# crowsonkb/style_transfer

Hardware: AMD Instinct MI355X
Metric: tile-iterations/sec, VGG-19 2048px/1024-tile (fwd+bwd, Gram/content losses, regularizers, Adam step) (higher is better)
Workload: dtype f32 (fp16x2-split MFMA, fp32 accumulate)

## Files before the change

### style_transfer_amd/build.py

```python

import concurrent.futures
import os
import subprocess
import sys

CSRC = os.path.join(os.path.dirname(os.path.abspath(__file__)), 'csrc')
REPO = os.path.dirname(os.path.dirname(os.path.abspath(__file__)))
INCLUDE = os.path.join(REPO, 'include')
LIB = os.path.join(CSRC, 'libstx.so')
HIPCC = os.environ.get('HIPCC', '/opt/rocm/bin/hipcc')
ARCH = 'gfx950'

SOURCES = {
    'conv_mfma.hip': [],
    'conv_wino2.hip': [],
    'conv_first.hip': [],
    'conv_h2.hip': [],
    'gram.hip': [],
    'symm.hip': [],
    'pool.hip': [],
    'reduce.hip': [],
    'content_mask.hip': [],
    'image_ops.hip': ['-ffp-contract=off'],
    'swt.hip': ['-ffp-contract=off'],
    'style_mask.hip': ['-ffp-contract=off'],
    'lap.hip': ['-ffp-contract=off'],
    'stat.hip': ['-ffp-contract=off'],
    'conv_dispatch.cpp': [],
    'engine.cpp': [],
    'tile_path.cpp': [],
    'image_api.cpp': [],
    'op_hooks.cpp': [],
}
EXTRA = os.environ.get('STX_HIPCC_EXTRA', '').split()
COMMON = EXTRA + ['--offload-arch=' + ARCH, '-O3', '-std=c++17', '-fPIC', '-I' + INCLUDE, '-I' + CSRC,
          '-Wall', '-Wno-unused-function']


def _stale(target, deps):
    if not os.path.exists(target):
        return True
    t = os.path.getmtime(target)
    return any(os.path.getmtime(d) > t for d in deps)


def _compile(src, extra, force):
    obj = os.path.join(CSRC, os.path.splitext(src)[0] + '.o')
    path = os.path.join(CSRC, src)
    deps = [path, os.path.join(CSRC, 'common.h'), os.path.join(CSRC, 'bf16x3.h'),
            os.path.join(CSRC, 'f16x2.h'), os.path.join(CSRC, 'engine.h'), os.path.join(INCLUDE, 'stx.h')]
    if force or _stale(obj, deps):
        cmd = [HIPCC] + COMMON + extra + ['-c', path, '-o', obj]
        proc = subprocess.run(cmd, stdout=subprocess.PIPE, stderr=subprocess.STDOUT, text=True)
        if proc.returncode != 0:
            raise RuntimeError('hipcc failed on %s:\n%s' % (src, proc.stdout))
        if proc.stdout.strip():
            sys.stderr.write(proc.stdout)
    return obj


def build(force=False, verbose=False):
    with concurrent.futures.ThreadPoolExecutor(max_workers=len(SOURCES)) as ex:
        futs = [ex.submit(_compile, src, extra, force) for src, extra in SOURCES.items()]
        objs = [f.result() for f in futs]
    if force or _stale(LIB, objs):
        cmd = [HIPCC, '--offload-arch=' + ARCH, '-shared', '-fPIC', '-o', LIB] + objs
        proc = subprocess.run(cmd, stdout=subprocess.PIPE, stderr=subprocess.STDOUT, text=True)
        if proc.returncode != 0:
            raise RuntimeError('link failed:\n' + proc.stdout)
    if verbose:
        print('built', LIB)
    return LIB


if __name__ == '__main__':
    build(force='--force' in sys.argv, verbose=True)
```

### style_transfer_amd/csrc/common.h

```cpp
#pragma once

#include <hip/hip_runtime.h>

#include <vector>

#include <cstdarg>
#include <cstdio>
#include <functional>
#include <string>

#include "stx.h"

namespace stx {

constexpr float kEps = 1.1920928955078125e-07f;

void set_error(const char *fmt, ...);

const char *sw_env(const char *name);
void sw_reread();

#define STX_HIP(call)                                                                       \
    do {                                                                                    \
        hipError_t err__ = (call);                                                          \
// ... 205 lines not shown
int wino2_splitk_factor(const ConvConfig &cfg, const ConvProblem &p);
struct Wino2Tail { int items, slices; };
Wino2Tail wino2_tail_split(const ConvConfig &cfg, const ConvProblem &p);
int wino2_max_slices(const ConvConfig &cfg, const ConvProblem &p);

constexpr int kAmaxSlots = 64;
ConvConfig h2_config(int mb, int pb = 1);
ConvConfig h2_pick_config(const ConvProblem &p);
bool h2_usable(const ConvProblem &p);
size_t h2_packed_floats(int K, int M);
int h2_pack_weights(hipStream_t s, const float *w_caffe, int Mo, int Ko, int transpose_flip, float *packed);
int h2_launch(hipStream_t s, const ConvConfig &cfg, const ConvProblem &p, int ksplit);
int h2_splitk_factor(const ConvConfig &cfg, const ConvProblem &p);
bool h2_fuses_pool(const ConvProblem &p);
bool h2_takes_pooled_input(const ConvConfig &cfg, const ConvProblem &p);
int absmax_launch(hipStream_t s, const float *x, size_t n, unsigned *slots);

size_t conv_small_packed_floats(int K);
int conv_small_pack(hipStream_t s, const float *w_caffe, int Mo, int Ko, int transpose_flip,
                    float *packed);
int conv_small_launch(hipStream_t s, const float *x, const float *packed, float *y,
                      const float *mask, int K, int M, int H, int W);

bool conv_h2_enabled();
struct ConvTuner { int device; hipStream_t stream; hipEvent_t ev0, ev1; std::function<int(const ConvConfig &, const float **)> bank; };
int conv_choose(const ConvProblem &p, bool winograd, const ConvTuner *tuner, ConvConfig *out);
struct ConvBank { int key; size_t floats; std::function<int(hipStream_t, const float *w_caffe, float *packed)> pack; };
ConvBank conv_bank(const ConvConfig &cfg, int dir, int Mo, int Ko, int ksize);
ConvBank conv_small_bank(int Mo, int Ko);
int conv_dispatch(hipStream_t s, const ConvConfig &cfg, const ConvProblem &p, double *flop_algorithmic,
                  double *flop_issued);
int conv_splitk_factor(const ConvConfig &cfg, const ConvProblem &p);
size_t conv_splitk_floats(const ConvConfig &cfg, const ConvProblem &p);
bool conv_takes_clock(const ConvConfig &cfg);
bool conv_fuses_pool(const ConvConfig &cfg, const ConvProblem &p);
bool conv_writes_pool_codes(const ConvConfig &cfg);
bool conv_reads_x_amax(const ConvConfig &cfg);
bool conv_leaves_y_amax(const ConvConfig &cfg);
bool conv_takes_inject(const ConvConfig &cfg);
bool conv_takes_pooled_input(const ConvConfig &cfg, const ConvProblem &p);
bool conv_uses_relu_codes(const ConvConfig &cfg, const ConvProblem &p, int ksplit);
bool conv_writes_out_codes(const ConvConfig &cfg, const ConvProblem &p, int ksplit);

int pool_forward_launch(hipStream_t s, const float *x, int C, int H, int W, int mode, float *y,
                        unsigned char *codes = nullptr);
int pool_backward_codes_launch(hipStream_t s, const float *dy, const unsigned char *codes, int C,
                               int H, int W, int mode, bool relu_mask, float *dx);
int pool_backward_launch(hipStream_t s, const float *dy, const float *x, int C, int H, int W,
                         int mode, bool relu_mask, float *dx);

struct GramPlan {
    int C, HW, splits, tiles;
    int parts;
    size_t partial_floats;
};
GramPlan gram_plan(int C, int HW);
bool gram_h2_usable(const float *feat, int C, int HW);
int gram_partials_launch(hipStream_t s, const float *feat, const GramPlan &plan, float *partials,
                         const unsigned *f_amax = nullptr);
int gram_finish_blocks(const GramPlan &plan);
int gram_finish_launch(hipStream_t s, const float *partials, const GramPlan &plan, float *gram_out,
                       const float *target, float *dsym, float *sumsq, unsigned short *pieces = nullptr,
                       const unsigned *f_amax = nullptr, float *block_out = nullptr);

size_t symm_pieces_elems(int C);
int symm_num_workgroups(int C, int HW);
bool symm_bf3_usable(const float *feat, const float *out, int C, int HW);
bool symm_h2_usable(const float *feat, const float *out, int C, int HW);
int symm_h2_launch(hipStream_t s, const float *feat, const float *dsym, const unsigned *d_amax, int n_damax,
                   const unsigned *f_amax, float *out, float *partials, int C, int HW);
int symm_bf3_launch(hipStream_t s, const float *feat, const float *dsym, unsigned short *pieces,
                    bool pieces_ready, float *out, float *partials, int C, int HW);

#ifdef __HIPCC__
__device__ __forceinline__ int content_origin_y(const ContentWindow &w) { return w.oy - w.sy; }
__device__ __forceinline__ int content_origin_x(const ContentWindow &w) { return w.ox - w.sx; }
__device__ __forceinline__ size_t content_index(const ContentWindow &w, int c, int y, int x) {
    int yy = (content_origin_y(w) + y) % w.ch;
    int xx = (content_origin_x(w) + x) % w.cw;
    if (yy < 0) yy += w.ch;
    if (xx < 0) xx += w.cw;
    return ((size_t)c * w.ch + yy) * w.cw + xx;
}
#endif

struct SumJob {
    const float *src;
    int n;
    float *dst;
};
int sum_jobs_launch(hipStream_t s, const SumJob *jobs, int n_jobs);
int content_sums_launch(hipStream_t s, const float *feat, const float *content,
                        const ContentWindow &win, float *sums , std::vector<SumJob> *defer = nullptr);
int inject_style_launch(hipStream_t s, float *diff, const float *sgrad, size_t n,
                        const float *abs_sum, float coef, bool accumulate, unsigned *y_amax = nullptr);
int inject_content_launch(hipStream_t s, float *diff, const float *feat, const float *content,
                          const ContentWindow &win, const float *sums, float coef, bool accumulate,
                          unsigned *y_amax = nullptr);
int relu_inplace_launch(hipStream_t s, float *x, size_t n);
int sum_partials_launch(hipStream_t s, const float *partials, int n, float *out);
int sum_partials2_launch(hipStream_t s, const float *a, int na, float *out_a, const float *b, int nb,
                         float *out_b);

constexpr int kMaskParts = 1024;
constexpr int kMaskSgradParts = 2048;
int mask_map_launch(hipStream_t s, const float *mask, int H, int W, int scale, float *out);
int mask_apply_launch(hipStream_t s, const float *feat, const float *map, const ContentWindow &win, float *fm,
                      float *m2_partials, int *n_parts);
int mask_target_launch(hipStream_t s, const float *gs, int C, const float *m2_partials, int n_parts, int HW,
                       float *out, float *a_out);
int mask_sgrad_launch(hipStream_t s, float *sgrad, const float *map, const ContentWindow &win, const float *a,
                      float *partials, int *n_parts);

constexpr int kContentMaskParts = 1024;
int content_mask_mean_launch(hipStream_t s, const float *map, const ContentWindow &win, float *a_out);
int content_mask_term_launch(hipStream_t s, const float *feat, const float *content, const float *map,
                             const ContentWindow &win, const float *a, float *sgrad, float *partials,
                             int *n_parts);

constexpr int kStatSlice = 16384;
constexpr float kStatEps = 1e-5f;
// ... 82 lines not shown
```

### style_transfer_amd/csrc/gram.hip

```cpp

#include <algorithm>
#include <cstdlib>
#include <cstring>

#include "bf16x3.h"
#include "common.h"
#include "f16x2.h"

namespace stx {

typedef float f32x16 __attribute__((ext_vector_type(16)));

constexpr int kGT = 64;
constexpr int kGP = 64;
constexpr int kGLd = kGP + 1;

GramPlan gram_plan(int C, int HW) {
    GramPlan p;
    p.C = C;
    p.HW = HW;
    const int T = ceil_div(C, kGT);
    p.tiles = T * (T + 1) / 2;
    int target = 512, min_stages = 8;
    if (const char *env = sw_env("STX_GRAM_WGS")) target = std::max(1, atoi(env));
    if (const char *env = sw_env("STX_GRAM_MIN_STAGES")) min_stages = std::max(1, atoi(env));
    int splits = std::max(1, target / p.tiles);
    splits = std::min(splits, ceil_div(HW, min_stages * kGP));
    splits = std::max(splits, 1);
    p.splits = splits;
    p.parts = 1;
    p.partial_floats = (size_t)p.splits * p.parts * p.tiles * kGT * kGT;
    return p;
}

__device__ __forceinline__ void tile_coords(int tile, int &ti, int &tj) {
    int r = (int)((sqrtf(8.f * tile + 1.f) - 1.f) * 0.5f);
    while ((r + 1) * (r + 2) / 2 <= tile) ++r;
    while (r * (r + 1) / 2 > tile) --r;
    ti = r;
    tj = tile - r * (r + 1) / 2;
}

template <bool VEC4>
__global__ __launch_bounds__(256, 2) void gram_partial_kernel(const float *__restrict__ F, int C,
                                                              int HW, int tiles, int slice,
                                                              int parts,
                                                              float *__restrict__ partials) {
    __shared__ float At[kGT * kGLd];
    __shared__ float Bt[kGT * kGLd];
    const int tid = threadIdx.x, lane = tid & 63;
    const int wave = __builtin_amdgcn_readfirstlane(tid >> 6);
    const int l31 = lane & 31, half = lane >> 5;
    const int tile = blockIdx.x % tiles, split = blockIdx.x / tiles;
    int ti, tj;
    tile_coords(tile, ti, tj);
    const bool diag = ti == tj;
    const int p_begin = split * slice;
    const int p_end = min(HW, p_begin + slice);
    const int bi = wave >> 1, bj = wave & 1;

    f32x16 acc;
#pragma unroll
    for (int r = 0; r < 16; ++r) acc[r] = 0.f;

    float ra[16], rb[16];
    auto load = [&](int p0) {
        if (VEC4) {
#pragma unroll
            for (int n = 0; n < 4; ++n) {
                const int e = tid + 256 * n;
                const int ch = e >> 4, px = p0 + (e & 15) * 4;
                const int ca = ti * kGT + ch, cb = tj * kGT + ch;
                const bool okp = px < p_end;
                const bool oka = okp && ca < C, okb = okp && cb < C && !diag;
                const float4 va = *reinterpret_cast<const float4 *>(F + (oka ? (size_t)ca * HW + px : 0));
                const float4 vb = *reinterpret_cast<const float4 *>(F + (okb ? (size_t)cb * HW + px : 0));
                ra[4 * n + 0] = oka ? va.x : 0.f;
                ra[4 * n + 1] = oka ? va.y : 0.f;
                ra[4 * n + 2] = oka ? va.z : 0.f;
                ra[4 * n + 3] = oka ? va.w : 0.f;
                rb[4 * n + 0] = okb ? vb.x : 0.f;
                rb[4 * n + 1] = okb ? vb.y : 0.f;
                rb[4 * n + 2] = okb ? vb.z : 0.f;
                rb[4 * n + 3] = okb ? vb.w : 0.f;
            }
        } else {
#pragma unroll
            for (int n = 0; n < 16; ++n) {
                const int e = tid + 256 * n;
                const int ch = e >> 6, px = p0 + (e & 63);
                const int ca = ti * kGT + ch, cb = tj * kGT + ch;
                const bool okp = px < p_end;
                const bool oka = okp && ca < C, okb = okp && cb < C && !diag;
// ... 420 lines not shown
        if (p_begin + kGP < p_end) load(p_begin + kGP);
        __syncthreads();
        int buf = 0;
        for (int p0 = p_begin; p0 < p_end; p0 += kGP, buf ^= 1) {
            const float *base = lds + buf * kStageFloats;
            f16x8h ah[2], al[2], bh[2], bl[2];
            fragment(base + a_off, ah[0], al[0]);
            fragment(base + a_off + 32 * kGLdW, ah[1], al[1]);
            if (!diag) {
                fragment(base + b_off, bh[0], bl[0]);
                fragment(base + b_off + 32 * kGLdW, bh[1], bl[1]);
            }
            if (p0 + kGP < p_end) store(p0 + kGP, buf ^ 1);
            if (p0 + 2 * kGP < p_end) load(p0 + 2 * kGP);
#pragma unroll
            for (int i = 0; i < 2; ++i)
#pragma unroll
                for (int j = 0; j < 2; ++j) {
                    if (diag && j > i) continue;
                    acc[i][j] = mfma_split3(ah[i], al[i], diag ? ah[j] : bh[j], diag ? al[j] : bl[j], acc[i][j]);
                }
            __syncthreads();
        }
    }
    float *red = lds + wave * (kGT * kGT);
#pragma unroll
    for (int i = 0; i < 2; ++i)
#pragma unroll
        for (int j = 0; j < 2; ++j)
#pragma unroll
            for (int r = 0; r < 16; ++r) {
                const int row = i * 32 + (r & 3) + 8 * (r >> 2) + 4 * half;
                red[row * kGT + j * 32 + l31] = acc[i][j][r];
            }
    __syncthreads();
    static_assert(4 * kGT * kGT <= 2 * kStageFloats, "the four partial tiles must fit the stage buffers");
    float *out = partials + ((size_t)split * tiles + tile) * (kGT * kGT);
#pragma unroll
    for (int n = 0; n < 4; ++n) {
        const int e = tid + 256 * n;
        const float4 w0 = reinterpret_cast<const float4 *>(lds)[e];
        const float4 w1 = reinterpret_cast<const float4 *>(lds + kGT * kGT)[e];
        const float4 w2 = reinterpret_cast<const float4 *>(lds + 2 * kGT * kGT)[e];
        const float4 w3 = reinterpret_cast<const float4 *>(lds + 3 * kGT * kGT)[e];
        float4 v;
        v.x = ((w0.x + w1.x) + w2.x) + w3.x;
        v.y = ((w0.y + w1.y) + w2.y) + w3.y;
        v.z = ((w0.z + w1.z) + w2.z) + w3.z;
        v.w = ((w0.w + w1.w) + w2.w) + w3.w;
        reinterpret_cast<float4 *>(out)[e] = v;
    }
}

static bool gram_use_bf3() {
    const char *env = sw_env("STX_GRAM");
    return !(env && !strcmp(env, "fp32"));
}

bool gram_h2_usable(const float *feat, int C, int HW) {
    const char *env = sw_env("STX_GRAM");
    if (env && (!strcmp(env, "fp32") || !strcmp(env, "bf3"))) return false;
    return (reinterpret_cast<uintptr_t>(feat) & 3) == 0 && 4.0 * C * (double)HW < 2147483648.0;
}

int gram_partials_launch(hipStream_t s, const float *feat, const GramPlan &plan, float *partials,
                         const unsigned *f_amax) {
    int slice = ceil_div(plan.HW, plan.splits);
    slice = ceil_div(slice, kGP) * kGP;
    const bool aligned = (reinterpret_cast<uintptr_t>(feat) & 15) == 0;
    const double bytes = 4.0 * plan.C * (double)plan.HW;
    if (f_amax) {
        gram_partial_h2_kernel<<<plan.tiles * plan.splits, 256, 0, s>>>(
            feat, plan.C, plan.HW, plan.tiles, slice, (unsigned)bytes, f_amax, partials);
        STX_CHECK_LAUNCH();
        return STX_OK;
    }
    if ((reinterpret_cast<uintptr_t>(feat) & 3) == 0 && bytes < 2147483648.0 && gram_use_bf3()) {
        gram_partial_bf3_kernel<<<plan.tiles * plan.splits, 256, 0, s>>>(
            feat, plan.C, plan.HW, plan.tiles, slice, (unsigned)bytes, partials);
        STX_CHECK_LAUNCH();
        return STX_OK;
    }
    if ((reinterpret_cast<uintptr_t>(feat) & 3) == 0 && bytes < 2147483648.0 && !sw_env("STX_GRAM_NARROW")) {
        gram_partial_wide_kernel<<<plan.tiles * plan.splits, 256, 0, s>>>(
            feat, plan.C, plan.HW, plan.tiles, slice, (unsigned)bytes, partials);
        STX_CHECK_LAUNCH();
        return STX_OK;
    }
    if (plan.parts > 1)
        STX_HIP(hipMemsetAsync(partials, 0, plan.partial_floats * sizeof(float), s));
    if (plan.HW % 4 == 0 && aligned)
        gram_partial_kernel<true><<<plan.tiles * plan.splits, 256, 0, s>>>(
            feat, plan.C, plan.HW, plan.tiles, slice, plan.parts, partials);
    else
        gram_partial_kernel<false><<<plan.tiles * plan.splits, 256, 0, s>>>(
            feat, plan.C, plan.HW, plan.tiles, slice, plan.parts, partials);
    STX_CHECK_LAUNCH();
    return STX_OK;
}

__global__ __launch_bounds__(256) void gram_finish_kernel(const float *__restrict__ partials, int C,
                                                          int tiles, int splits, float scale,
                                                          float *__restrict__ gram,
                                                          const float *__restrict__ target,
                                                          float *__restrict__ dsym,
                                                          float *__restrict__ block_sumsq,
                                                          unsigned short *__restrict__ pieces,
                                                          const unsigned *__restrict__ f_amax,
                                                          unsigned *__restrict__ block_amax) {
    __shared__ float lane_sum[4][64];
    __shared__ float red[64];
    __shared__ float redm[64];
    float unscale = 1.f;
    if (f_amax) unscale = pow2f(-h2_scale_exp(amax_of_slots(f_amax, kAmaxSlots)));
    const int el = threadIdx.x & 63, sl = threadIdx.x >> 6;
    const int idx = blockIdx.x * 64 + el;
    const bool valid = idx < C * C;
    int i = 0, j = 0;
    float sum = 0.f;
    if (valid) {
        i = idx / C;
        j = idx % C;
    }
// ... 156 lines not shown
```

### style_transfer_amd/csrc/symm.hip

```cpp

#include <algorithm>
#include <cstdlib>
#include <cstring>

#include "bf16x3.h"
#include "common.h"
#include "f16x2.h"

#ifndef STX_SYMM_SKIP
#define STX_SYMM_SKIP 0
#endif

namespace stx {

namespace {

constexpr int kSM = 64;
constexpr int kSN = 256;
#ifndef STX_SYMM_KSK
#define STX_SYMM_KSK 32
#endif
constexpr int kSK = STX_SYMM_KSK;
constexpr int kSPC = kSK / 16;
constexpr int kSegs = kSK / 8;
// ... 132 lines not shown
                acc[i][j] = mfma_split6(pa[i], pb[j], acc[i][j]);
            }
    };

    int step = 0;
    auto advance = [&](int slot_) {
        const int chunk = step / kSPC, s_in = step % kSPC, buf = chunk & 1;
        if (step + kRing - 1 < n_steps && !(STX_SYMM_SKIP & 4)) f_load(step + kRing - 1, (slot_ + kRing - 1) % kRing);
        do_step(step, slot_, buf, s_in);
        if (s_in == kSPC - 1) {
            if (chunk + 1 < n_chunks) d_store(buf ^ 1);
            if (chunk + 2 < n_chunks) d_load(chunk + 2);
            __syncthreads();
        }
        ++step;
    };
    while (step < n_steps) {
#pragma unroll
        for (int r = 0; r < kRing; ++r)
            if (step < n_steps) advance(r);
    }

    float asum = 0.f;
#pragma unroll
    for (int i = 0; i < 2; ++i)
#pragma unroll
        for (int r = 0; r < 16; ++r) {
            const int row = m0 + i * 32 + (r & 3) + 8 * (r >> 2) + 4 * g;
            const int row0 = min(__builtin_amdgcn_readfirstlane(m0 + i * 32 + (r & 3) + 8 * (r >> 2)), C);
            const unsigned so = BIG ? 0u : (unsigned)row0 * HW4;
            const int rows_left = C - row0 < 5 ? C - row0 : 5;
            const __amdgpu_buffer_rsrc_t rrow =
                BIG ? __builtin_amdgcn_make_buffer_rsrc(S + (size_t)row0 * (size_t)HW, 0,
                                                        (rows_left > 0 ? rows_left : 0) * HW * 4, 0x00020000)
                    : rs;
#pragma unroll
            for (int j = 0; j < 2; ++j) {
                const int px = px0 + j * 32 + l31;
                const bool ok = row < C && px < HW;
                const float v = acc[i][j][r];
                asum += ok ? fabsf(v) : 0.f;
                const unsigned vo = ok ? (unsigned)((4 * g) * HW + px) * 4u : kOob;
                if (!(STX_SYMM_SKIP & 8))
                    __builtin_amdgcn_raw_buffer_store_b32(__builtin_bit_cast(unsigned, v), rrow, vo, so, 0);
            }
        }
#pragma unroll
    for (int off = 32; off > 0; off >>= 1) asum += __shfl_down(asum, off, 64);
    if (lane == 0) wave_sum[wave] = asum;
    __syncthreads();
    if (tid == 0) partials[blockIdx.x] = ((wave_sum[0] + wave_sum[1]) + wave_sum[2]) + wave_sum[3];
}

constexpr int kHChunkBytes = 2 * kPieceBytes;
constexpr int kHDLoads = kSM * kSK / 4 / 256;

template <bool BIG>
__global__ __launch_bounds__(256, 2) void symm_h2_kernel(const float *__restrict__ F,
                                                         const float *__restrict__ D,
                                                         const unsigned *__restrict__ d_amax, int n_damax,
                                                         const unsigned *__restrict__ f_amax,
                                                         float *__restrict__ S,
                                                         float *__restrict__ partials, int C, int Cp,
                                                         int HW, unsigned f_bytes, int m_tiles) {
    __shared__ __attribute__((aligned(16))) unsigned char lds[2 * kHChunkBytes];
    __shared__ float wave_sum[4];
    __shared__ unsigned wave_max[4];
    const int tid = threadIdx.x, lane = tid & 63;
    const int wave = __builtin_amdgcn_readfirstlane(tid >> 6);
    const int l31 = lane & 31, g = lane >> 5;
    const int nb = gridDim.x, xcd = blockIdx.x & 7, slot = blockIdx.x >> 3;
    const int q8 = nb >> 3, r8 = nb & 7;
    const int L = (xcd < r8 ? xcd * (q8 + 1) : r8 * (q8 + 1) + (xcd - r8) * q8) + slot;
    const int mt = __builtin_amdgcn_readfirstlane(L % m_tiles), pt = __builtin_amdgcn_readfirstlane(L / m_tiles);
    const int m0 = mt * kSM;
    const int px0 = pt * kSN + wave * 64;

    constexpr unsigned kOob = 0x80000000u;
    const __amdgpu_buffer_rsrc_t rf =
        __builtin_amdgcn_make_buffer_rsrc(const_cast<float *>(F), 0, BIG ? 0 : f_bytes, 0x00020000);
    const __amdgpu_buffer_rsrc_t rs = __builtin_amdgcn_make_buffer_rsrc(S, 0, BIG ? 0 : f_bytes, 0x00020000);
    const __amdgpu_buffer_rsrc_t rd =
        __builtin_amdgcn_make_buffer_rsrc(const_cast<float *>(D), 0, (unsigned)(C * C) * 4u, 0x00020000);
    unsigned voff[2];
#pragma unroll
    for (int j = 0; j < 2; ++j) {
        const int px = px0 + j * 32 + l31;
        voff[j] = px < HW ? (unsigned)((g * 8) * HW + px) * 4u : kOob;
    }
    const unsigned HW4 = (unsigned)HW * 4u;
    const int n_steps = Cp / 16, n_chunks = Cp / kSK;

    unsigned dvoff[kHDLoads], ddst[kHDLoads];
    int dcol[kHDLoads];
#pragma unroll
    for (int n = 0; n < kHDLoads; ++n) {
        const int e = tid + 256 * n;
        const int row = e / (kSK / 4), seg = e - row * (kSK / 4);
        dcol[n] = seg * 4;
        dvoff[n] = m0 + row < C ? (unsigned)((m0 + row) * C + seg * 4) * 4u : kOob;
        ddst[n] = (unsigned)(row * kRowBytes + seg * 8);
    }
    u32x4y dreg[kHDLoads];
    auto d_load = [&](int chunk) {
        const unsigned so = (unsigned)__builtin_amdgcn_readfirstlane(chunk * kSK * 4);
#pragma unroll
        for (int n = 0; n < kHDLoads; ++n)
            dreg[n] = __builtin_amdgcn_raw_buffer_load_b128(rd, dcol[n] + chunk * kSK < C ? dvoff[n] : kOob, so, 0);
    };

    float raw[kRing][2][8];
    auto f_load = [&](int step, int slot_) {
        const int k0 = __builtin_amdgcn_readfirstlane(step * 16);
        const int left = C - k0 < 16 ? C - k0 : 16;
        const __amdgpu_buffer_rsrc_t rk =
            BIG ? __builtin_amdgcn_make_buffer_rsrc(const_cast<float *>(F) + (size_t)k0 * (size_t)HW, 0,
                                                    (left > 0 ? left : 0) * HW * 4, 0x00020000)
                : rf;
#pragma unroll
        for (int j = 0; j < 2; ++j)
#pragma unroll
            for (int e = 0; e < 8; ++e)
                raw[slot_][j][e] = __builtin_bit_cast(
                    float, __builtin_amdgcn_raw_buffer_load_b32(
                               rk, voff[j], BIG ? (unsigned)e * HW4 : (unsigned)min(k0 + e, C) * HW4, 0));
    };

    f32x16h acc[2][2];
#pragma unroll
    for (int i = 0; i < 2; ++i)
#pragma unroll
        for (int j = 0; j < 2; ++j)
#pragma unroll
            for (int r = 0; r < 16; ++r) acc[i][j][r] = 0.f;

    d_load(0);
#pragma unroll
    for (int r = 0; r < kRing - 1; ++r)
        if (r < n_steps) f_load(r, r);

    const int ef = h2_scale_exp(amax_of_slots(f_amax, kAmaxSlots));
    unsigned dm = 0;
    for (int i = tid; i < n_damax; i += 256) dm = max(dm, d_amax[i]);
#pragma unroll
    for (int off = 32; off > 0; off >>= 1) dm = max(dm, (unsigned)__shfl_xor((int)dm, off, 64));
    if (lane == 0) wave_max[wave] = dm;
    __syncthreads();
    dm = max(max(wave_max[0], wave_max[1]), max(wave_max[2], wave_max[3]));
    const int ed = __builtin_amdgcn_readfirstlane(h2_scale_exp(dm));
    const float sf = pow2f(ef), sd = pow2f(ed);

    auto d_store = [&](int buf) {
#pragma unroll
        for (int n = 0; n < kHDLoads; ++n) {
            unsigned h[2], l[2];
            const unsigned d0 = dreg[n].x, d1 = dreg[n].y, d2 = dreg[n].z, d3 = dreg[n].w;
            split2_f16_quad(__builtin_bit_cast(float, d0), __builtin_bit_cast(float, d1),
                            __builtin_bit_cast(float, d2), __builtin_bit_cast(float, d3), sd, h, l);
            typedef unsigned u32x2s __attribute__((ext_vector_type(2)));
            unsigned char *q = lds + buf * kHChunkBytes + ddst[n];
            *reinterpret_cast<u32x2s *>(q) = (u32x2s){h[0], h[1]};
            *reinterpret_cast<u32x2s *>(q + kPieceBytes) = (u32x2s){l[0], l[1]};
        }
    };
    d_store(0);
    if (n_chunks > 1) d_load(1);
    __syncthreads();

    const unsigned a_off = (unsigned)(l31 * kRowBytes + g * 16);
    auto do_step = [&](int slot_, int buf, int s_in_chunk) {
        f16x8h bh[2], bl[2], ah[2], al[2];
#pragma unroll
        for (int j = 0; j < 2; ++j) split2_f16(raw[slot_][j], sf, bh[j], bl[j]);
        const unsigned char *base = lds + buf * kHChunkBytes + a_off + s_in_chunk * 32;
#pragma unroll
        for (int i = 0; i < 2; ++i) {
            ah[i] = *reinterpret_cast<const f16x8h *>(base + i * 32 * kRowBytes);
            al[i] = *reinterpret_cast<const f16x8h *>(base + kPieceBytes + i * 32 * kRowBytes);
        }
#pragma unroll
        for (int i = 0; i < 2; ++i)
#pragma unroll
            for (int j = 0; j < 2; ++j) acc[i][j] = mfma_split3(ah[i], al[i], bh[j], bl[j], acc[i][j]);
    };

    int step = 0;
    auto advance = [&](int slot_) {
        const int chunk = step / kSPC, s_in = step % kSPC, buf = chunk & 1;
        if (step + kRing - 1 < n_steps) f_load(step + kRing - 1, (slot_ + kRing - 1) % kRing);
        do_step(slot_, buf, s_in);
        if (s_in == kSPC - 1) {
            if (chunk + 1 < n_chunks) d_store(buf ^ 1);
            if (chunk + 2 < n_chunks) d_load(chunk + 2);
            __syncthreads();
        }
        ++step;
    };
    while (step < n_steps) {
#pragma unroll
        for (int r = 0; r < kRing; ++r)
            if (step < n_steps) advance(r);
    }

    const float ud = pow2f(-ed), uf = pow2f(-ef);
    float asum = 0.f;
#pragma unroll
    for (int i = 0; i < 2; ++i)
#pragma unroll
        for (int r = 0; r < 16; ++r) {
            const int row = m0 + i * 32 + (r & 3) + 8 * (r >> 2) + 4 * g;
            const int row0 = min(__builtin_amdgcn_readfirstlane(m0 + i * 32 + (r & 3) + 8 * (r >> 2)), C);
            const unsigned so = BIG ? 0u : (unsigned)row0 * HW4;
            const int rows_left = C - row0 < 5 ? C - row0 : 5;
            const __amdgpu_buffer_rsrc_t rrow =
                BIG ? __builtin_amdgcn_make_buffer_rsrc(S + (size_t)row0 * (size_t)HW, 0,
                                                        (rows_left > 0 ? rows_left : 0) * HW * 4, 0x00020000)
                    : rs;
#pragma unroll
            for (int j = 0; j < 2; ++j) {
                const int px = px0 + j * 32 + l31;
                const bool ok = row < C && px < HW;
                const float v = (acc[i][j][r] * ud) * uf;
                asum += ok ? fabsf(v) : 0.f;
                const unsigned vo = ok ? (unsigned)((4 * g) * HW + px) * 4u : kOob;
                __builtin_amdgcn_raw_buffer_store_b32(__builtin_bit_cast(unsigned, v), rrow, vo, so, 0);
            }
        }
#pragma unroll
    for (int off = 32; off > 0; off >>= 1) asum += __shfl_down(asum, off, 64);
    if (lane == 0) wave_sum[wave] = asum;
    __syncthreads();
    if (tid == 0) partials[blockIdx.x] = ((wave_sum[0] + wave_sum[1]) + wave_sum[2]) + wave_sum[3];
}

__global__ void symm_split_kernel(const float *__restrict__ dsym, int C, int Cp,
                                  unsigned short *__restrict__ pieces) {
    const int idx = blockIdx.x * blockDim.x + threadIdx.x;
    if (idx >= Cp * Cp) return;
    const int i = idx / Cp, j = idx - i * Cp;
    unsigned short s1 = 0, s2 = 0, s3 = 0;
    if (i < C && j < C) split3_bf16_scalar(dsym[i * C + j], s1, s2, s3);
    pieces[idx] = s1;
    pieces[(size_t)Cp * Cp + idx] = s2;
    pieces[2 * (size_t)Cp * Cp + idx] = s3;
}

int symm_num_workgroups(int C, int HW) { return ceil_div(C, kSM) * ceil_div(HW, kSN); }

bool symm_bf3_usable(const float *feat, const float *out, int C, int HW) {
    const char *env = sw_env("STX_SYMM");
    if (env && !strcmp(env, "fp32")) return false;
    return 64.0 * (double)HW < 2147483648.0 &&
           ((reinterpret_cast<uintptr_t>(feat) | reinterpret_cast<uintptr_t>(out)) & 3) == 0;
}

int symm_bf3_launch(hipStream_t s, const float *feat, const float *dsym, unsigned short *pieces,
                    bool pieces_ready, float *out, float *partials, int C, int HW) {
    const int Cp = ceil_div(C, kSM) * kSM;
    if (!pieces_ready || Cp != C) {
        symm_split_kernel<<<ceil_div(Cp * Cp, 256), 256, 0, s>>>(dsym, C, Cp, pieces);
        STX_CHECK_LAUNCH();
    }
    const int m_tiles = Cp / kSM;
    const double bytes = 4.0 * C * (double)HW;
    const char *force_big = sw_env("STX_WINO_BIG");
    if (bytes >= 2147483648.0 || (force_big && atoi(force_big) == 1))
        symm_bf3_kernel<true><<<symm_num_workgroups(C, HW), 256, 0, s>>>(feat, pieces, out, partials, C, Cp,
                                                                       HW, 0u, m_tiles);
    else
        symm_bf3_kernel<false><<<symm_num_workgroups(C, HW), 256, 0, s>>>(feat, pieces, out, partials, C, Cp,
                                                                        HW, (unsigned)bytes, m_tiles);
    STX_CHECK_LAUNCH();
    return STX_OK;
}

bool symm_h2_usable(const float *feat, const float *out, int C, int HW) {
    const char *env = sw_env("STX_SYMM");
    if (env && (!strcmp(env, "fp32") || !strcmp(env, "bf3"))) return false;
    return C % 4 == 0 && symm_bf3_usable(feat, out, C, HW);
}

int symm_h2_launch(hipStream_t s, const float *feat, const float *dsym, const unsigned *d_amax, int n_damax,
                   const unsigned *f_amax, float *out, float *partials, int C, int HW) {
    const int Cp = ceil_div(C, kSM) * kSM;
    const int m_tiles = Cp / kSM;
    const double bytes = 4.0 * C * (double)HW;
    const char *force_big = sw_env("STX_WINO_BIG");
    if (bytes >= 2147483648.0 || (force_big && atoi(force_big) == 1))
        symm_h2_kernel<true><<<symm_num_workgroups(C, HW), 256, 0, s>>>(feat, dsym, d_amax, n_damax, f_amax, out,
                                                                      partials, C, Cp, HW, 0u, m_tiles);
    else
        symm_h2_kernel<false><<<symm_num_workgroups(C, HW), 256, 0, s>>>(feat, dsym, d_amax, n_damax, f_amax, out,
                                                                       partials, C, Cp, HW, (unsigned)bytes, m_tiles);
    STX_CHECK_LAUNCH();
    return STX_OK;
}

}
```

### style_transfer_amd/csrc/tile_path.cpp

```cpp

#include <algorithm>
#include <cmath>
#include <cstdlib>
#include <deque>

#include "engine.h"

namespace stx {

ConvProblem conv_fwd_problem(const float *x, float *y, const float *bias, int Cin, int Cout, int H, int W,
                             int ks, int relu) {
    ConvProblem p{};
    p.x = x;
    p.y = y;
    p.bias = bias;
    p.K = Cin;
    p.M = Cout;
    p.H = H;
    p.W = W;
    p.ksize = ks;
    p.relu = relu;
    p.epilogue = kEpiForward;
    return p;
}
// ... 298 lines not shown
    ProfScope scope(e, "bwd " + L.name, conv_flops(cp.cout, cp.cin, b.h, b.w, cp.ks));
    return launch_conv(e, cfg, p);
}

static size_t style_term_scratch_floats(int C, int HW) {
    return 2 * (size_t)ceil_div(C * C, 64) + (size_t)symm_num_workgroups(C, HW) + 64;
}

int launch_style_terms(stx_engine *e, hipStream_t stream, const float *feat, int C, int h, int w,
                       const float *target, float *sgrad, float *sc, const std::string &name,
                       const unsigned *f_amax, float *term_scratch, std::vector<SumJob> *defer) {
    const int HW = h * w;
    const bool fused = e->first_gram_valid && e->first_gram_blob >= 0 &&
                       feat == e->blobs[e->first_gram_blob].data.f() && C == 64;
    GramPlan plan = gram_plan(C, HW);
    if (fused) {
        plan.splits = e->first_gram_parts;
        plan.tiles = 1;
        plan.parts = 1;
        plan.partial_floats = (size_t)plan.splits * 64 * 64;
    }
    const int fin_blocks = gram_finish_blocks(plan);
    float *const partials = fused ? e->first_gram.f() : nullptr;
    if (!fused) STX_TRY(e->gram_partials.ensure((plan.partial_floats + 2 * fin_blocks) * sizeof(float)));
    STX_TRY(e->dsym.ensure((size_t)C * C * sizeof(float)));
    const bool gram_h2 = !fused && gram_h2_usable(feat, C, HW);
    const bool symm_h2 = symm_h2_usable(feat, sgrad, C, HW);
    const bool bf3 = !symm_h2 && symm_bf3_usable(feat, sgrad, C, HW);
    if ((gram_h2 || symm_h2) && !f_amax) {
        unsigned *scratch;
        STX_TRY(amax_scratch(e, &scratch));
        ProfScope scope(e, "absmax " + name, 0.0, stream);
        STX_TRY(absmax_launch(stream, feat, (size_t)C * HW, scratch));
        f_amax = scratch;
    }
    if (bf3) STX_TRY(e->dsym_pieces.ensure(symm_pieces_elems(C) * sizeof(unsigned short)));
    unsigned short *pieces = bf3 && C % 64 == 0 ? static_cast<unsigned short *>(e->dsym_pieces.ptr) : nullptr;
    {
        ProfScope scope(e, "gram " + name, 2.0 * C * C * (double)HW, stream);
        if (!fused) STX_TRY(gram_partials_launch(stream, feat, plan, e->gram_partials.f(), gram_h2 ? f_amax : nullptr));
        STX_TRY(gram_finish_launch(stream, fused ? partials : e->gram_partials.f(), plan, nullptr, target,
                                   e->dsym.f(), nullptr, pieces, gram_h2 ? f_amax : nullptr,
                                   defer ? term_scratch : nullptr));
    }
    ProfScope scope(e, "symm " + name, 2.0 * C * C * (double)HW, stream);
    const float *block_sumsq = defer ? term_scratch : (fused ? partials : e->gram_partials.f()) + plan.partial_floats;
    auto finish = [&](float *symm_partials, int n_wg) -> int {
        if (!defer) return sum_partials2_launch(stream, block_sumsq, fin_blocks, sc, symm_partials, n_wg, sc + 1);
        defer->push_back(SumJob{block_sumsq, fin_blocks, sc});
        defer->push_back(SumJob{symm_partials, n_wg, sc + 1});
        return STX_OK;
    };
    if (symm_h2 || bf3) {
        const int n_wg = symm_num_workgroups(C, HW);
        float *symm_partials = defer ? term_scratch + 2 * fin_blocks : nullptr;
        if (!defer) {
            STX_TRY(e->symm_partials.ensure((size_t)n_wg * sizeof(float)));
            symm_partials = e->symm_partials.f();
        }
        if (symm_h2)
            STX_TRY(symm_h2_launch(stream, feat, e->dsym.f(), reinterpret_cast<const unsigned *>(block_sumsq + fin_blocks),
                                   fin_blocks, f_amax, sgrad, symm_partials, C, HW));
        else
            STX_TRY(symm_bf3_launch(stream, feat, e->dsym.f(), static_cast<unsigned short *>(e->dsym_pieces.ptr),
                                    pieces != nullptr, sgrad, symm_partials, C, HW));
        return finish(symm_partials, n_wg);
    }
    const ConvConfig cfg = conv_pick_config(1, C, C, h, w);
    const int n_wg = conv_num_workgroups(cfg, C, h, w);
    STX_TRY(e->symm_partials.ensure((size_t)n_wg * sizeof(float)));
    ConvProblem p{};
    p.x = feat;
    p.w = e->dsym.f();
    p.y = sgrad;
    p.partials = e->symm_partials.f();
    p.K = C;
    p.M = C;
    p.H = h;
    p.W = w;
    p.ksize = 1;
    p.epilogue = kEpiSymm;
    STX_TRY(conv_launch(stream, cfg, p, false));
    return sum_partials2_launch(stream, block_sumsq, fin_blocks, sc, e->symm_partials.f(), n_wg, sc + 1);
}

int launch_masked_style_terms(stx_engine *e, hipStream_t stream, const float *feat, int C, int h, int w,
                              const float *mask_map, const ContentWindow &win, const float *target,
                              float *sgrad, float *sc, const std::string &name, const unsigned *f_amax,
                              float *term_scratch, float *mask_scratch, std::vector<SumJob> *defer) {
    STX_TRY(e->masked_feat.ensure((size_t)C * h * w * sizeof(float)));
    STX_TRY(e->masked_target.ensure((size_t)C * C * sizeof(float)));
    float *const m2_partials = mask_scratch, *const ms_partials = mask_scratch + kMaskParts;
    {
        ProfScope scope(e, "mask " + name, 0.0, stream);
        int n_m2 = 0;
        STX_TRY(mask_apply_launch(stream, feat, mask_map, win, e->masked_feat.f(), m2_partials, &n_m2));
        STX_TRY(mask_target_launch(stream, target, C, m2_partials, n_m2, h * w, e->masked_target.f(), sc + 3));
    }
    STX_TRY(launch_style_terms(e, stream, e->masked_feat.f(), C, h, w, e->masked_target.f(), sgrad, sc, name,
                               f_amax, term_scratch, defer));
    ProfScope scope(e, "smask " + name, 0.0, stream);
    int n_ms = 0;
    STX_TRY(mask_sgrad_launch(stream, sgrad, mask_map, win, sc + 3, ms_partials, &n_ms));
    if (!defer) return sum_partials_launch(stream, ms_partials, n_ms, sc + 2);
    defer->push_back(SumJob{ms_partials, n_ms, sc + 2});
    return STX_OK;
}
// ... 730 lines not shown
```

Baseline: 270.9.

## Add 128-wide super-tiles for Gram partials and symm h2 kernel

Adds an optional Gram partial kernel where each 512-thread workgroup computes a 128x128 super-tile (up to four 64x64 output tiles) from shared LDS panels, enabled only by an environment variable. It also templates the symm h2 kernel on its M tile size and, by default for large channel counts and pixel counts, uses 128-row tiles. The intent is to reuse each loaded feature panel across more output rows and cut global/LDS traffic per MFMA. The cost is more accumulator registers and LDS per workgroup, which may lower occupancy or cause spills.

```diff
diff --git a/style_transfer_amd/build.py b/style_transfer_amd/build.py
--- a/style_transfer_amd/build.py
+++ b/style_transfer_amd/build.py
@@ -48,7 +48,7 @@
     obj = os.path.join(CSRC, os.path.splitext(src)[0] + '.o')
     path = os.path.join(CSRC, src)
     deps = [path, os.path.join(CSRC, 'common.h'), os.path.join(CSRC, 'bf16x3.h'),
-            os.path.join(CSRC, 'f16x2.h'), os.path.join(CSRC, 'engine.h'), os.path.join(INCLUDE, 'stx.h')]
+            os.path.join(CSRC, 'f16x2.h'), os.path.join(CSRC, 'gram_tiles.h'), os.path.join(CSRC, 'engine.h'), os.path.join(INCLUDE, 'stx.h')]
     if force or _stale(obj, deps):
         cmd = [HIPCC] + COMMON + extra + ['-c', path, '-o', obj]
         proc = subprocess.run(cmd, stdout=subprocess.PIPE, stderr=subprocess.STDOUT, text=True)
diff --git a/style_transfer_amd/csrc/common.h b/style_transfer_amd/csrc/common.h
--- a/style_transfer_amd/csrc/common.h
+++ b/style_transfer_amd/csrc/common.h
@@ -281,6 +281,7 @@
 struct GramPlan {
     int C, HW, splits, tiles;
     int parts;
+    int tile;
     size_t partial_floats;
 };
 GramPlan gram_plan(int C, int HW);
@@ -296,6 +297,7 @@
 int symm_num_workgroups(int C, int HW);
 bool symm_bf3_usable(const float *feat, const float *out, int C, int HW);
 bool symm_h2_usable(const float *feat, const float *out, int C, int HW);
+int symm_h2_num_workgroups(int C, int HW);
 int symm_h2_launch(hipStream_t s, const float *feat, const float *dsym, const unsigned *d_amax, int n_damax,
                    const unsigned *f_amax, float *out, float *partials, int C, int HW);
 int symm_bf3_launch(hipStream_t s, const float *feat, const float *dsym, unsigned short *pieces,
diff --git a/style_transfer_amd/csrc/gram.hip b/style_transfer_amd/csrc/gram.hip
--- a/style_transfer_amd/csrc/gram.hip
+++ b/style_transfer_amd/csrc/gram.hip
@@ -6,6 +6,7 @@
 #include "bf16x3.h"
 #include "common.h"
 #include "f16x2.h"
+#include "gram_tiles.h"
 
 namespace stx {
 
@@ -14,6 +15,14 @@
 constexpr int kGT = 64;
 constexpr int kGP = 64;
 constexpr int kGLd = kGP + 1;
+
+static bool gram_super_wanted(int C, int HW) {
+    const char *tile = sw_env("STX_GRAM_TILE");
+    if (!tile || atoi(tile) != 128) return false;
+    const char *env = sw_env("STX_GRAM");
+    if (env && (!strcmp(env, "fp32") || !strcmp(env, "bf3"))) return false;
+    return C > kGT && 4.0 * C * (double)HW < 2147483648.0;
+}
 
 GramPlan gram_plan(int C, int HW) {
     GramPlan p;
@@ -21,10 +30,12 @@
     p.HW = HW;
     const int T = ceil_div(C, kGT);
     p.tiles = T * (T + 1) / 2;
-    int target = 512, min_stages = 8;
+    p.tile = gram_super_wanted(C, HW) ? 2 * kGT : kGT;
+    const bool super = p.tile > kGT;
+    int target = super ? 256 : 512, min_stages = 8;
     if (const char *env = sw_env("STX_GRAM_WGS")) target = std::max(1, atoi(env));
     if (const char *env = sw_env("STX_GRAM_MIN_STAGES")) min_stages = std::max(1, atoi(env));
-    int splits = std::max(1, target / p.tiles);
+    int splits = std::max(1, target / (super ? gram_super_tiles(T) : p.tiles));
     splits = std::min(splits, ceil_div(HW, min_stages * kGP));
     splits = std::max(splits, 1);
     p.splits = splits;
@@ -34,11 +45,7 @@
 }
 
 __device__ __forceinline__ void tile_coords(int tile, int &ti, int &tj) {
-    int r = (int)((sqrtf(8.f * tile + 1.f) - 1.f) * 0.5f);
-    while ((r + 1) * (r + 2) / 2 <= tile) ++r;
-    while (r * (r + 1) / 2 > tile) --r;
-    ti = r;
-    tj = tile - r * (r + 1) / 2;
+    tri_coords(tile, ti, tj);
 }
 
 template <bool VEC4>
@@ -565,6 +572,173 @@
     }
 }
 
+constexpr int kGPanel = 2 * kGT * kGLdW;
+constexpr int kGSStage = 2 * kGPanel;
+constexpr size_t kGSLdsBytes = 2 * kGSStage * sizeof(float);
+
+__global__ __launch_bounds__(512, 1) void gram_partial_h2s_kernel(const float *__restrict__ F, int C, int HW,
+                                                                  int T, int tiles, int stiles, int slice,
+                                                                  unsigned f_bytes,
+                                                                  const unsigned *__restrict__ f_amax,
+                                                                  float *__restrict__ partials) {
+    extern __shared__ __attribute__((aligned(16))) float lds[];
+    const int tid = threadIdx.x, lane = tid & 63;
+    const int wave8 = __builtin_amdgcn_readfirstlane(tid >> 6);
+    const int grp = wave8 >> 2, wave = wave8 & 3;
+    const int l31 = lane & 31, half = lane >> 5;
+    const int nb = gridDim.x, xcd = blockIdx.x & 7, slot = blockIdx.x >> 3;
+    const int q8 = nb >> 3, r8 = nb & 7;
+    const int L = (xcd < r8 ? xcd * (q8 + 1) : r8 * (q8 + 1) + (xcd - r8) * q8) + slot;
+    const int st = __builtin_amdgcn_readfirstlane(L % stiles), split = __builtin_amdgcn_readfirstlane(L / stiles);
+    int si, sj;
+    tri_coords(st, si, sj);
+    si = __builtin_amdgcn_readfirstlane(si);
+    sj = __builtin_amdgcn_readfirstlane(sj);
+    const bool diag = si == sj;
+    const int p_begin = split * slice;
+    const int p_end = min(HW, p_begin + slice);
+    int ti, tjs[2], tile_of[2];
+#pragma unroll
+    for (int t = 0; t < 2; ++t)
+        tile_of[t] = __builtin_amdgcn_readfirstlane(gram_super_member(st, grp, t, T, ti, tjs[t]));
+    ti = __builtin_amdgcn_readfirstlane(ti);
+    const bool tdiag[2] = {tile_of[0] >= 0 && 2 * sj == ti, tile_of[1] >= 0 && 2 * sj + 1 == ti};
+
+    f32x16 acc[2][2][2];
+#pragma unroll
+    for (int t = 0; t < 2; ++t)
+#pragma unroll
+        for (int i = 0; i < 2; ++i)
+#pragma unroll
+            for (int j = 0; j < 2; ++j)
+#pragma unroll
+                for (int r = 0; r < 16; ++r) acc[t][i][j][r] = 0.f;
+
+    constexpr unsigned kOob = 0x80000000u;
+    const __amdgpu_buffer_rsrc_t rf =
+        __builtin_amdgcn_make_buffer_rsrc(const_cast<float *>(F), 0, f_bytes, 0x00020000);
+    unsigned aoff[4], boff[4];
+    int ldst[4];
+#pragma unroll
+    for (int n = 0; n < 4; ++n) {
+        const int e = tid + 512 * n;
+        const int ch = e >> 4, px = (e & 15) * 4;
+        const int ca = si * 2 * kGT + ch, cb = sj * 2 * kGT + ch;
+        aoff[n] = ca < C ? (unsigned)(ca * HW + px) * 4u : kOob;
+        boff[n] = cb < C && !diag ? (unsigned)(cb * HW + px) * 4u : kOob;
+        ldst[n] = ch * kGLdW + px;
+    }
+    u32x4g ra[4], rb[4];
+    auto load = [&](int p0) {
+        const unsigned so = (unsigned)__builtin_amdgcn_readfirstlane(p0 * 4);
+#pragma unroll
+        for (int n = 0; n < 4; ++n) ra[n] = __builtin_amdgcn_raw_buffer_load_b128(rf, aoff[n], so, 0);
+        if (!diag) {
+#pragma unroll
+            for (int n = 0; n < 4; ++n) rb[n] = __builtin_amdgcn_raw_buffer_load_b128(rf, boff[n], so, 0);
+        }
+    };
+    auto store = [&](int p0, int buf) {
+        float *At = lds + buf * kGSStage, *Bt = At + kGPanel;
+#pragma unroll
+        for (int n = 0; n < 4; ++n) {
+            const int rem = p_end - (p0 + ((tid + 512 * n) & 15) * 4);
+            u32x4g va = ra[n], vb = rb[n];
+            if (rem < 4) {
+                va.x = rem > 0 ? va.x : 0u, va.y = rem > 1 ? va.y : 0u, va.z = rem > 2 ? va.z : 0u, va.w = 0u;
+                vb.x = rem > 0 ? vb.x : 0u, vb.y = rem > 1 ? vb.y : 0u, vb.z = rem > 2 ? vb.z : 0u, vb.w = 0u;
+            }
+            *reinterpret_cast<u32x4g *>(At + ldst[n]) = va;
+            if (!diag) *reinterpret_cast<u32x4g *>(Bt + ldst[n]) = vb;
+        }
+    };
+
+    const int f_off = l31 * kGLdW + wave * 16 + half * 8;
+    const int a_off = grp * kGT * kGLdW + f_off;
+    const int b_off = (diag ? 0 : kGPanel) + f_off;
+    const float sv = pow2f(h2_scale_exp(amax_of_slots(f_amax, kAmaxSlots)));
+    auto fragment = [&](const float *q, f16x8h &hi, f16x8h &lo) {
+        const f32x4g v0 = *reinterpret_cast<const f32x4g *>(q);
+        const f32x4g v1 = *reinterpret_cast<const f32x4g *>(q + 4);
+        const float x[8] = {v0.x, v0.y, v0.z, v0.w, v1.x, v1.y, v1.z, v1.w};
+        split2_f16(x, sv, hi, lo);
+    };
+
+    if (p_begin < p_end) {
+        load(p_begin);
+        store(p_begin, 0);
+        if (p_begin + kGP < p_end) load(p_begin + kGP);
+        __syncthreads();
+        int buf = 0;
+        for (int p0 = p_begin; p0 < p_end; p0 += kGP, buf ^= 1) {
+            const float *base = lds + buf * kGSStage;
+            f16x8h ah[2], al[2];
+            if (tile_of[0] >= 0) {
+                fragment(base + a_off, ah[0], al[0]);
+                fragment(base + a_off + 32 * kGLdW, ah[1], al[1]);
+            }
+            if (p0 + kGP < p_end) store(p0 + kGP, buf ^ 1);
+            if (p0 + 2 * kGP < p_end) load(p0 + 2 * kGP);
+#pragma unroll
+            for (int t = 0; t < 2; ++t) {
+                if (tile_of[t] < 0) continue;
+                f16x8h bh[2], bl[2];
+                if (tdiag[t]) {
+                    bh[0] = ah[0], bl[0] = al[0], bh[1] = ah[1], bl[1] = al[1];
+                } else {
+                    fragment(base + b_off + t * kGT * kGLdW, bh[0], bl[0]);
+                    fragment(base + b_off + (t * kGT + 32) * kGLdW, bh[1], bl[1]);
+                }
+#pragma unroll
+                for (int i = 0; i < 2; ++i)
+#pragma unroll
+                    for (int j = 0; j < 2; ++j) {
+                        if (tdiag[t] && j > i) continue;
+                        acc[t][i][j] = mfma_split3(ah[i], al[i], bh[j], bl[j], acc[t][i][j]);
+                    }
+            }
+            __syncthreads();
+        }
+    }
+    static_assert(8 * kGT * kGT <= 2 * kGSStage, "the eight partial tiles must fit the stage buffers");
+    float *gred = lds + grp * 4 * (kGT * kGT);
+    const int gtid = tid & 255;
+#pragma unroll
+    for (int t = 0; t < 2; ++t) {
+        if (tile_of[t] >= 0) {
+            float *red = gred + wave * (kGT * kGT);
+#pragma unroll
+            for (int i = 0; i < 2; ++i)
+#pragma unroll
+                for (int j = 0; j < 2; ++j)
+#pragma unroll
+                    for (int r = 0; r < 16; ++r) {
+                        const int row = i * 32 + (r & 3) + 8 * (r >> 2) + 4 * half;
+                        red[row * kGT + j * 32 + l31] = acc[t][i][j][r];
+                    }
+        }
+        __syncthreads();
+        if (tile_of[t] >= 0) {
+            float *out = partials + ((size_t)split * tiles + tile_of[t]) * (kGT * kGT);
+#pragma unroll
+            for (int n = 0; n < 4; ++n) {
+                const int e = gtid + 256 * n;
+                const float4 w0 = reinterpret_cast<const float4 *>(gred)[e];
+                const float4 w1 = reinterpret_cast<const float4 *>(gred + kGT * kGT)[e];
+                const float4 w2 = reinterpret_cast<const float4 *>(gred + 2 * kGT * kGT)[e];
+                const float4 w3 = reinterpret_cast<const float4 *>(gred + 3 * kGT * kGT)[e];
+                float4 v;
+                v.x = ((w0.x + w1.x) + w2.x) + w3.x;
+                v.y = ((w0.y + w1.y) + w2.y) + w3.y;
+                v.z = ((w0.z + w1.z) + w2.z) + w3.z;
+                v.w = ((w0.w + w1.w) + w2.w) + w3.w;
+                reinterpret_cast<float4 *>(out)[e] = v;
+            }
+        }
+        __syncthreads();
+    }
+}
+
 static bool gram_use_bf3() {
     const char *env = sw_env("STX_GRAM");
     return !(env && !strcmp(env, "fp32"));
@@ -582,6 +756,19 @@
     slice = ceil_div(slice, kGP) * kGP;
     const bool aligned = (reinterpret_cast<uintptr_t>(feat) & 15) == 0;
     const double bytes = 4.0 * plan.C * (double)plan.HW;
+    if (f_amax && plan.tile > kGT) {
+        const int T = ceil_div(plan.C, kGT), stiles = gram_super_tiles(T);
+        hipError_t err = hipFuncSetAttribute(reinterpret_cast<const void *>(gram_partial_h2s_kernel),
+                                             hipFuncAttributeMaxDynamicSharedMemorySize, (int)kGSLdsBytes);
+        if (err != hipSuccess) {
+            set_error("hipFuncSetAttribute(lds=%zu): %s", kGSLdsBytes, hipGetErrorString(err));
+            return STX_ERR_HIP;
+        }
+        gram_partial_h2s_kernel<<<stiles * plan.splits, 512, kGSLdsBytes, s>>>(
+            feat, plan.C, plan.HW, T, plan.tiles, stiles, slice, (unsigned)bytes, f_amax, partials);
+        STX_CHECK_LAUNCH();
+        return STX_OK;
+    }
     if (f_amax) {
         gram_partial_h2_kernel<<<plan.tiles * plan.splits, 256, 0, s>>>(
             feat, plan.C, plan.HW, plan.tiles, slice, (unsigned)bytes, f_amax, partials);
diff --git a/style_transfer_amd/csrc/gram_tiles.h b/style_transfer_amd/csrc/gram_tiles.h
--- /dev/null
+++ b/style_transfer_amd/csrc/gram_tiles.h
@@ -0,0 +1,35 @@
+#pragma once
+
+#include <math.h>
+
+#ifdef __HIPCC__
+#define STX_HD __host__ __device__
+#else
+#define STX_HD
+#endif
+
+namespace stx {
+
+STX_HD inline void tri_coords(int idx, int &i, int &j) {
+    int r = (int)((sqrtf(8.f * idx + 1.f) - 1.f) * 0.5f);
+    while ((r + 1) * (r + 2) / 2 <= idx) ++r;
+    while (r * (r + 1) / 2 > idx) --r;
+    i = r;
+    j = idx - r * (r + 1) / 2;
+}
+
+STX_HD inline int gram_super_tiles(int T) {
+    const int T2 = (T + 1) / 2;
+    return T2 * (T2 + 1) / 2;
+}
+
+STX_HD inline int gram_super_member(int st, int g, int t, int T, int &ti, int &tj) {
+    int si, sj;
+    tri_coords(st, si, sj);
+    ti = 2 * si + g;
+    tj = 2 * sj + t;
+    if (ti >= T || tj > ti) return -1;
+    return ti * (ti + 1) / 2 + tj;
+}
+
+}
diff --git a/style_transfer_amd/csrc/symm.hip b/style_transfer_amd/csrc/symm.hip
--- a/style_transfer_amd/csrc/symm.hip
+++ b/style_transfer_amd/csrc/symm.hip
@@ -208,10 +208,7 @@
     if (tid == 0) partials[blockIdx.x] = ((wave_sum[0] + wave_sum[1]) + wave_sum[2]) + wave_sum[3];
 }
 
-constexpr int kHChunkBytes = 2 * kPieceBytes;
-constexpr int kHDLoads = kSM * kSK / 4 / 256;
-
-template <bool BIG>
+template <bool BIG, int MT = kSM>
 __global__ __launch_bounds__(256, 2) void symm_h2_kernel(const float *__restrict__ F,
                                                          const float *__restrict__ D,
                                                          const unsigned *__restrict__ d_amax, int n_damax,
@@ -219,8 +216,12 @@
                                                          float *__restrict__ S,
                                                          float *__restrict__ partials, int C, int Cp,
                                                          int HW, unsigned f_bytes, int m_tiles) {
+    constexpr int kMB = MT / 32;
+    constexpr int kPieceBytesT = MT * kRowBytes;
+    constexpr int kHChunkBytes = 2 * kPieceBytesT;
+    constexpr int kHDLoads = MT * kSK / 4 / 256;
     __shared__ __attribute__((aligned(16))) unsigned char lds[2 * kHChunkBytes];
-    __shared__ float wave_sum[4];
+    __shared__ float wave_sum[MT / kSM][4];
     __shared__ unsigned wave_max[4];
     const int tid = threadIdx.x, lane = tid & 63;
     const int wave = __builtin_amdgcn_readfirstlane(tid >> 6);
@@ -229,7 +230,7 @@
     const int q8 = nb >> 3, r8 = nb & 7;
     const int L = (xcd < r8 ? xcd * (q8 + 1) : r8 * (q8 + 1) + (xcd - r8) * q8) + slot;
     const int mt = __builtin_amdgcn_readfirstlane(L % m_tiles), pt = __builtin_amdgcn_readfirstlane(L / m_tiles);
-    const int m0 = mt * kSM;
+    const int m0 = mt * MT;
     const int px0 = pt * kSN + wave * 64;
 
     constexpr unsigned kOob = 0x80000000u;
@@ -282,9 +283,9 @@
                                rk, voff[j], BIG ? (unsigned)e * HW4 : (unsigned)min(k0 + e, C) * HW4, 0));
     };
 
-    f32x16h acc[2][2];
-#pragma unroll
-    for (int i = 0; i < 2; ++i)
+    f32x16h acc[kMB][2];
+#pragma unroll
+    for (int i = 0; i < kMB; ++i)
 #pragma unroll
         for (int j = 0; j < 2; ++j)
 #pragma unroll
@@ -316,7 +317,7 @@
             typedef unsigned u32x2s __attribute__((ext_vector_type(2)));
             unsigned char *q = lds + buf * kHChunkBytes + ddst[n];
             *reinterpret_cast<u32x2s *>(q) = (u32x2s){h[0], h[1]};
-            *reinterpret_cast<u32x2s *>(q + kPieceBytes) = (u32x2s){l[0], l[1]};
+            *reinterpret_cast<u32x2s *>(q + kPieceBytesT) = (u32x2s){l[0], l[1]};
         }
     };
     d_store(0);
@@ -325,17 +326,17 @@
 
     const unsigned a_off = (unsigned)(l31 * kRowBytes + g * 16);
     auto do_step = [&](int slot_, int buf, int s_in_chunk) {
-        f16x8h bh[2], bl[2], ah[2], al[2];
+        f16x8h bh[2], bl[2], ah[kMB], al[kMB];
 #pragma unroll
         for (int j = 0; j < 2; ++j) split2_f16(raw[slot_][j], sf, bh[j], bl[j]);
         const unsigned char *base = lds + buf * kHChunkBytes + a_off + s_in_chunk * 32;
 #pragma unroll
-        for (int i = 0; i < 2; ++i) {
+        for (int i = 0; i < kMB; ++i) {
             ah[i] = *reinterpret_cast<const f16x8h *>(base + i * 32 * kRowBytes);
-            al[i] = *reinterpret_cast<const f16x8h *>(base + kPieceBytes + i * 32 * kRowBytes);
-        }
-#pragma unroll
-        for (int i = 0; i < 2; ++i)
+            al[i] = *reinterpret_cast<const f16x8h *>(base + kPieceBytesT + i * 32 * kRowBytes);
+        }
+#pragma unroll
+        for (int i = 0; i < kMB; ++i)
 #pragma unroll
             for (int j = 0; j < 2; ++j) acc[i][j] = mfma_split3(ah[i], al[i], bh[j], bl[j], acc[i][j]);
     };
@@ -359,9 +360,11 @@
     }
 
     const float ud = pow2f(-ed), uf = pow2f(-ef);
-    float asum = 0.f;
-#pragma unroll
-    for (int i = 0; i < 2; ++i)
+    float hsum[MT / kSM];
+#pragma unroll
+    for (int i = 0; i < kMB; ++i) {
+        if (i % 2 == 0) hsum[i / 2] = 0.f;
+        float &asum = hsum[i / 2];
 #pragma unroll
         for (int r = 0; r < 16; ++r) {
             const int row = m0 + i * 32 + (r & 3) + 8 * (r >> 2) + 4 * g;
@@ -382,11 +385,20 @@
                 __builtin_amdgcn_raw_buffer_store_b32(__builtin_bit_cast(unsigned, v), rrow, vo, so, 0);
             }
         }
-#pragma unroll
-    for (int off = 32; off > 0; off >>= 1) asum += __shfl_down(asum, off, 64);
-    if (lane == 0) wave_sum[wave] = asum;
+    }
+#pragma unroll
+    for (int hf = 0; hf < MT / kSM; ++hf) {
+        float asum = hsum[hf];
+#pragma unroll
+        for (int off = 32; off > 0; off >>= 1) asum += __shfl_down(asum, off, 64);
+        if (lane == 0) wave_sum[hf][wave] = asum;
+    }
     __syncthreads();
-    if (tid == 0) partials[blockIdx.x] = ((wave_sum[0] + wave_sum[1]) + wave_sum[2]) + wave_sum[3];
+    if (tid == 0) {
+        float total = ((wave_sum[0][0] + wave_sum[0][1]) + wave_sum[0][2]) + wave_sum[0][3];
+        if (MT > kSM) total += ((wave_sum[MT / kSM - 1][0] + wave_sum[MT / kSM - 1][1]) + wave_sum[MT / kSM - 1][2]) + wave_sum[MT / kSM - 1][3];
+        partials[blockIdx.x] = total;
+    }
 }
 
 __global__ void symm_split_kernel(const float *__restrict__ dsym, int C, int Cp,
@@ -436,18 +448,33 @@
     return C % 4 == 0 && symm_bf3_usable(feat, out, C, HW);
 }
 
+static int symm_h2_tile(int C, int HW) {
+    const char *force_big = sw_env("STX_WINO_BIG");
+    if (C < 2 * kSM || 4.0 * C * (double)HW >= 2147483648.0 || (force_big && atoi(force_big) == 1)) return kSM;
+    if (const char *tile = sw_env("STX_SYMM_TILE")) {
+        if (atoi(tile) == kSM) return kSM;
+        if (atoi(tile) == 2 * kSM) return 2 * kSM;
+    }
+    return C >= 4 * kSM && ceil_div(C, 2 * kSM) * ceil_div(HW, kSN) >= 512 ? 2 * kSM : kSM;
+}
+
+int symm_h2_num_workgroups(int C, int HW) { return ceil_div(C, symm_h2_tile(C, HW)) * ceil_div(HW, kSN); }
+
 int symm_h2_launch(hipStream_t s, const float *feat, const float *dsym, const unsigned *d_amax, int n_damax,
                    const unsigned *f_amax, float *out, float *partials, int C, int HW) {
     const int Cp = ceil_div(C, kSM) * kSM;
-    const int m_tiles = Cp / kSM;
+    const int mt = symm_h2_tile(C, HW), m_tiles = ceil_div(C, mt), n_wg = symm_h2_num_workgroups(C, HW);
     const double bytes = 4.0 * C * (double)HW;
     const char *force_big = sw_env("STX_WINO_BIG");
     if (bytes >= 2147483648.0 || (force_big && atoi(force_big) == 1))
-        symm_h2_kernel<true><<<symm_num_workgroups(C, HW), 256, 0, s>>>(feat, dsym, d_amax, n_damax, f_amax, out,
-                                                                      partials, C, Cp, HW, 0u, m_tiles);
+        symm_h2_kernel<true><<<n_wg, 256, 0, s>>>(feat, dsym, d_amax, n_damax, f_amax, out,
+                                                  partials, C, Cp, HW, 0u, m_tiles);
+    else if (mt > kSM)
+        symm_h2_kernel<false, 2 * kSM><<<n_wg, 256, 0, s>>>(feat, dsym, d_amax, n_damax, f_amax, out,
+                                                            partials, C, Cp, HW, (unsigned)bytes, m_tiles);
     else
-        symm_h2_kernel<false><<<symm_num_workgroups(C, HW), 256, 0, s>>>(feat, dsym, d_amax, n_damax, f_amax, out,
-                                                                       partials, C, Cp, HW, (unsigned)bytes, m_tiles);
+        symm_h2_kernel<false><<<n_wg, 256, 0, s>>>(feat, dsym, d_amax, n_damax, f_amax, out,
+                                                   partials, C, Cp, HW, (unsigned)bytes, m_tiles);
     STX_CHECK_LAUNCH();
     return STX_OK;
 }
diff --git a/style_transfer_amd/csrc/tile_path.cpp b/style_transfer_amd/csrc/tile_path.cpp
--- a/style_transfer_amd/csrc/tile_path.cpp
+++ b/style_transfer_amd/csrc/tile_path.cpp
@@ -374,7 +374,7 @@
         return STX_OK;
     };
     if (symm_h2 || bf3) {
-        const int n_wg = symm_num_workgroups(C, HW);
+        const int n_wg = symm_h2 ? symm_h2_num_workgroups(C, HW) : symm_num_workgroups(C, HW);
         float *symm_partials = defer ? term_scratch + 2 * fin_blocks : nullptr;
         if (!defer) {
             STX_TRY(e->symm_partials.ensure((size_t)n_wg * sizeof(float)));
```

Result: no change. 270.0 (-0.3%).
